# k-flouris/cmf

Measured on AMD Instinct MI355X. Metric: log-density evals/sec (JtJ-cholesky path), MNIST D=784 d=64 bs=512, higher is better.
Workload: dtype f32 (3x3 tangent convs as bf16x3 split MFMA, fp32 accumulate); 1 GPU; C3: MNIST-shaped (1,28,28) uint8-range + U[0,1) noise, non-square flow d=64, cholesky J^T J log-det + g_ij off-diagonal L1 + reconstruction, eval/no_grad; per_gpu_batch=512, global_batch=512, D=784, latent_dimension=64, parallelism=dp1

## Files before the change

cmf_amd/csrc/probe_front.hip:

```cpp
#include <stdint.h>

#include "common.h"

namespace {

constexpr int HID = 64, NT = 256, SLICE = HID * 16;
constexpr int MAXT = 50;
constexpr int MAXCLS = 32;
constexpr int PASS = 64;

__global__ __launch_bounds__(NT) void probe_apply_kernel(cmf_probe_apply_args a, int nitems) {
  __shared__ __attribute__((aligned(16))) float Rs[MAXCLS * HID];
  __shared__ __attribute__((aligned(16))) float Ts[MAXT * PASS];
  __shared__ int tcls[MAXT], toff[MAXT];
  __shared__ int nterm;

  const int per = (nitems + 7) >> 3;
  const int item = (int)(blockIdx.x & 7) * per + (int)(blockIdx.x >> 3);
  if (item >= nitems) return;
  const int H = a.H, W = a.W, HW = H * W;
  const int b = item / HW, p = item - b * HW;
  const int tid = threadIdx.x, lane = tid & 63, wv = tid >> 6;
  const int ncls = a.ns * 16;
  const f32x4 zero = {0.f, 0.f, 0.f, 0.f};

  unsigned long long live = ~0ull;
  if (a.ymask)
    live = *reinterpret_cast<const unsigned long long*>(reinterpret_cast<const unsigned char*>(a.ymask) + (long long)b * a.ymask_np +
                                                        (long long)p * (HID / 8));

  if (wv == 0) {
    int cls = -1, off = 0;
    if (lane < 25 * a.cin) {
      const int w = lane / a.cin, c = lane - w * a.cin;
      const int r = p / W + w / 5 - 2, col = p % W + w % 5 - 2;
      if (r >= 0 && r < H && col >= 0 && col < W) {
        const int q = r * W + col, k = a.cls[c * HW + q];
        if (k >= 0 && k < ncls) {
          cls = k;
          off = (int)(c * a.t_c + q * a.t_px);
        }
      }
    }
    const unsigned long long bal = __ballot(cls >= 0);
    if (cls >= 0) {
      const int pos = __popcll(bal & ((1ull << lane) - 1ull));
      tcls[pos] = cls;
      toff[pos] = off;
    }
    if (lane == 0) nterm = __popcll(bal);
  }

  {
    const int co = tid >> 2, k4 = (tid & 3) * 4;
    const float* rb = a.r + (long long)b * a.r_np + (long long)p * a.r_px + tid * 4;
    for (int s = 0; s < a.ns; ++s) {
      f32x4 v = zero;
      if ((live >> co) & 1) v = *reinterpret_cast<const f32x4*>(rb + s * SLICE);
#pragma unroll
      for (int m = 0; m < 4; ++m) Rs[(s * 16 + k4 + m) * HID + (co & 15) * 4 + (co >> 4)] = v[m];
    }
  }
  __syncthreads();

  const int n = nterm, nsl = a.nc >> 4, cg = lane >> 2, quad = lane & 3;
  const float* tb = a.t + (long long)b * a.t_np;
  for (int s0 = 0; s0 < nsl; s0 += PASS / 16) {
    const int w4 = (nsl - s0 < PASS / 16 ? nsl - s0 : PASS / 16) * 4;
    if (s0) __syncthreads();
    for (int i = tid; i < n * w4; i += NT) {
      const int j = i / w4, x = i - j * w4;
      *reinterpret_cast<f32x4*>(&Ts[j * PASS + 4 * x]) = *reinterpret_cast<const f32x4*>(tb + toff[j] + s0 * 16 + 4 * x);
    }
    __syncthreads();
    const int sl = s0 + wv;
    if (sl >= nsl) continue;
    f32x4 acc[4] = {zero, zero, zero, zero};
    for (int j = 0; j < n; ++j) {
      const f32x4 c4 = *reinterpret_cast<const f32x4*>(&Rs[tcls[j] * HID + cg * 4]);
      const f32x4 t4 = *reinterpret_cast<const f32x4*>(&Ts[j * PASS + wv * 16 + quad * 4]);
#pragma unroll
      for (int i = 0; i < 4; ++i)
#pragma unroll
        for (int k = 0; k < 4; ++k) acc[i][k] = fmaf(c4[i], t4[k], acc[i][k]);
    }
    float* yb = a.y + (long long)b * a.y_np + (long long)p * a.y_px + sl * SLICE + quad * 4;
#pragma unroll
    for (int i = 0; i < 4; ++i) {
      const int co = cg + 16 * i;
      if ((live >> co) & 1) *reinterpret_cast<f32x4*>(yb + co * 16) = acc[i];
    }
  }
}

bool fits_i32(long long v) { return v >= 0 && v <= 0x7fffffffLL; }

}

extern "C" int cmf_probe_apply(const cmf_probe_apply_args* ap, void* stream) {
  if (!ap) return CMF_EINVAL;
  const cmf_probe_apply_args& a = *ap;
  if (!a.r || !a.t || !a.cls || !a.y) return CMF_EINVAL;
  if (a.np <= 0 || a.H <= 0 || a.W <= 0 || a.nc <= 0 || a.nc % 16) return CMF_EINVAL;
  if (a.cin < 1 || 25 * a.cin > MAXT || a.ns < 1 || a.ns * 16 > MAXCLS) return CMF_EINVAL;
  if ((a.r_np | a.r_px | a.t_np | a.t_c | a.t_px | a.y_np | a.y_px) % 4) return CMF_EINVAL;
  if ((uintptr_t)a.r % 16 || (uintptr_t)a.t % 16 || (uintptr_t)a.y % 16) return CMF_EINVAL;
  if (a.r_np < 0 || a.t_np < 0 || a.y_np < 0 || a.t_c < 0) return CMF_EINVAL;
  if (a.r_px < (long long)a.ns * SLICE || a.y_px < (long long)HID * a.nc || a.t_px < a.nc) return CMF_EINVAL;
  const long long HW = (long long)a.H * a.W;
  if (a.ymask && ((uintptr_t)a.ymask % 8 || a.ymask_np % 8 || a.ymask_np < HW * (HID / 8))) return CMF_EINVAL;
  if (HW > (1 << 24) || !fits_i32(a.cin * a.t_c + HW * a.t_px + a.nc)) return CMF_ERANGE;
  const long long nitems = HW * a.np;
  if (nitems > 0x7ffffff0LL) return CMF_ERANGE;
  const int grid = 8 * (int)((nitems + 7) / 8);
  hipLaunchKernelGGL(probe_apply_kernel, dim3(grid), dim3(NT), 0, (hipStream_t)stream, a, (int)nitems);
  CMF_LAUNCH_CHECK();
  return 0;
}
```

Baseline: 1510 evals/s.

## Process horizontal pixel strips per block with shared T band and per-wave pipelining

Restructures the probe-apply kernel so each block handles a strip of 8–16 pixels in a row for one 64-channel pass, instead of one pixel per block. The block loads the 5-row halo band of T and class ids into LDS once and shares it across the strip's pixels. Each wave prefetches the next pixel's R through buffer loads with masked offsets, iterates terms via ballot and readlane, and stores through buffer stores. The kernel is templated on cin/ns and gets occupancy launch bounds. This cuts redundant T/cls loads and per-pixel block overhead, at the cost of more LDS per block and more code complexity.

Result: no change. 1517 evals/s, median of 6 (+0.4%).

```diff
diff --git a/cmf_amd/csrc/probe_front.hip b/cmf_amd/csrc/probe_front.hip
--- a/cmf_amd/csrc/probe_front.hip
+++ b/cmf_amd/csrc/probe_front.hip
@@ -4,92 +4,196 @@
 
 namespace {
 
-constexpr int HID = 64, NT = 256, SLICE = HID * 16;
+constexpr int HID = 64, NT = 256, NW = NT / 64, SLICE = HID * 16;
 constexpr int MAXT = 50;
 constexpr int MAXCLS = 32;
 constexpr int PASS = 64;
-
-__global__ __launch_bounds__(NT) void probe_apply_kernel(cmf_probe_apply_args a, int nitems) {
-  __shared__ __attribute__((aligned(16))) float Rs[MAXCLS * HID];
-  __shared__ __attribute__((aligned(16))) float Ts[MAXT * PASS];
-  __shared__ int tcls[MAXT], toff[MAXT];
-  __shared__ int nterm;
+constexpr int RS_FLAGS = 0x00020000, DROP = 0x7ffffff0;
+constexpr int RROW = HID + 4;
+
+constexpr int strip_of(int cin) { return cin == 1 ? 16 : 8; }
+
+typedef unsigned long long u64;
+typedef unsigned bu32x4 __attribute__((vector_size(16)));
+
+__device__ __forceinline__ auto rsrc_of(const void* p, int bytes) {
+  const u64 u = reinterpret_cast<u64>(p);
+  const unsigned lo = __builtin_amdgcn_readfirstlane((int)(unsigned)u), hi = __builtin_amdgcn_readfirstlane((int)(unsigned)(u >> 32));
+  return __builtin_amdgcn_make_buffer_rsrc(reinterpret_cast<void*>(((u64)hi << 32) | lo), 0, bytes, RS_FLAGS);
+}
+
+__device__ __forceinline__ void wave_lds_fence() {
+  __builtin_amdgcn_fence(__ATOMIC_RELEASE, "wavefront");
+  __builtin_amdgcn_wave_barrier();
+  __builtin_amdgcn_fence(__ATOMIC_ACQUIRE, "wavefront");
+}
+
+__device__ __forceinline__ u64 lane_word(u64 v, int l) {
+  const unsigned lo = __builtin_amdgcn_readlane((int)(unsigned)v, l), hi = __builtin_amdgcn_readlane((int)(unsigned)(v >> 32), l);
+  return ((u64)hi << 32) | lo;
+}
+
+template <int NS>
+__device__ __forceinline__ void fetch_r(f32x4 (&rv)[4 * NS], const float* r, u64 live, bool on, int lane) {
+  const auto rs = rsrc_of(r, on ? NS * SLICE * 4 : 0);
+#pragma unroll
+  for (int s = 0; s < NS; ++s)
+#pragma unroll
+    for (int k = 0; k < 4; ++k)
+      rv[4 * s + k] = __builtin_bit_cast(f32x4, __builtin_amdgcn_raw_buffer_load_b128(
+          rs, (live >> (16 * k + (lane >> 2))) & 1 ? 4 * (s * SLICE + k * 256 + lane * 4) : DROP, 0, 0));
+}
+
+template <int NS>
+__device__ __forceinline__ void write_image(float* Rw, const f32x4 (&rv)[4 * NS], int lane) {
+#pragma unroll
+  for (int s = 0; s < NS; ++s)
+#pragma unroll
+    for (int m = 0; m < 4; ++m) {
+      const f32x4 v = {rv[4 * s][m], rv[4 * s + 1][m], rv[4 * s + 2][m], rv[4 * s + 3][m]};
+      *reinterpret_cast<f32x4*>(&Rw[(s * 16 + (lane & 3) * 4 + m) * RROW + (lane >> 2) * 4]) = v;
+    }
+}
+
+template <int NSL, int CIN, int NS>
+__device__ __forceinline__ void strip_pixels(float* Rw, const float* Tb, const int* bcls, f32x4 (&rv)[4 * NS], u64 words, const float* rb,
+                                             long long r_px, float* yb, long long y_px, int len, int wv, int lane) {
+  constexpr int BAND = strip_of(CIN) + 4;
+  const int cg = lane >> 2, quad = lane & 3;
+  const f32x4 zero = {0.f, 0.f, 0.f, 0.f};
+  write_image<NS>(Rw, rv, lane);
+  for (int x = wv; x < len; x += NW) {
+    const u64 live = lane_word(words, x);
+    const bool more = x + NW < len;
+    wave_lds_fence();
+    fetch_r<NS>(rv, rb + (more ? x + NW : x) * r_px, more ? lane_word(words, x + NW) : 0ull, more, lane);
+
+    int cls = -1, pos = 0;
+    if (lane < 25 * CIN) {
+      const int w = lane / CIN, c = lane - w * CIN;
+      pos = (c * 5 + w / 5) * BAND + x + w % 5;
+      cls = bcls[pos];
+    }
+    const u64 terms = __ballot(cls >= 0);
+
+    f32x4 acc[NSL][4], c4, t4[NSL];
+#pragma unroll
+    for (int s = 0; s < NSL; ++s)
+#pragma unroll
+      for (int i = 0; i < 4; ++i) acc[s][i] = zero;
+    auto read_term = [&](u64& m, f32x4& c, f32x4(&t)[NSL]) {
+      const int l = __builtin_ctzll(m);
+      const int k = __builtin_amdgcn_readlane(cls, l), o = __builtin_amdgcn_readlane(pos, l);
+      m &= m - 1;
+      c = *reinterpret_cast<const f32x4*>(&Rw[k * RROW + cg * 4]);
+#pragma unroll
+      for (int s = 0; s < NSL; ++s) t[s] = *reinterpret_cast<const f32x4*>(&Tb[o * PASS + s * 16 + quad * 4]);
+    };
+    auto add_term = [&]() {
+#pragma unroll
+      for (int s = 0; s < NSL; ++s)
+#pragma unroll
+        for (int i = 0; i < 4; ++i)
+#pragma unroll
+          for (int e = 0; e < 4; ++e) acc[s][i][e] = fmaf(c4[i], t4[s][e], acc[s][i][e]);
+    };
+    if (terms) {
+      u64 m = terms;
+      read_term(m, c4, t4);
+      while (m) {
+        f32x4 cn, tn[NSL];
+        read_term(m, cn, tn);
+        add_term();
+        c4 = cn;
+#pragma unroll
+        for (int s = 0; s < NSL; ++s) t4[s] = tn[s];
+      }
+      add_term();
+    }
+
+    const auto ys = rsrc_of(yb + x * y_px, NSL * SLICE * 4);
+#pragma unroll
+    for (int s = 0; s < NSL; ++s)
+#pragma unroll
+      for (int i = 0; i < 4; ++i) {
+        const int co = cg + 16 * i;
+        __builtin_amdgcn_raw_buffer_store_b128(__builtin_bit_cast(bu32x4, acc[s][i]), ys, (live >> co) & 1 ? 4 * (s * SLICE + co * 16 + quad * 4) : DROP, 0, 0);
+      }
+    wave_lds_fence();
+    write_image<NS>(Rw, rv, lane);
+  }
+}
+
+constexpr int wg_per_cu(int cin, int ns) {
+  return 160 * 1024 / (4 * (cin * 5 * (strip_of(cin) + 4) * (PASS + 1) + NW * 16 * ns * RROW));
+}
+
+template <int CIN, int NS>
+__global__ __launch_bounds__(NT, wg_per_cu(CIN, NS)) void probe_apply_kernel(cmf_probe_apply_args a, int nitems, int spr, int npass) {
+  constexpr int STRIP = strip_of(CIN), BAND = STRIP + 4;
+  constexpr int NPOS = CIN * 5 * BAND, NB = (NPOS + 15) / 16, NCLS = 16 * NS;
+  __shared__ __attribute__((aligned(16))) float Tb[NPOS * PASS];
+  __shared__ __attribute__((aligned(16))) float Rs[NW][NCLS * RROW];
+  __shared__ int bcls[NPOS];
 
   const int per = (nitems + 7) >> 3;
   const int item = (int)(blockIdx.x & 7) * per + (int)(blockIdx.x >> 3);
   if (item >= nitems) return;
   const int H = a.H, W = a.W, HW = H * W;
-  const int b = item / HW, p = item - b * HW;
-  const int tid = threadIdx.x, lane = tid & 63, wv = tid >> 6;
-  const int ncls = a.ns * 16;
-  const f32x4 zero = {0.f, 0.f, 0.f, 0.f};
-
-  unsigned long long live = ~0ull;
-  if (a.ymask)
-    live = *reinterpret_cast<const unsigned long long*>(reinterpret_cast<const unsigned char*>(a.ymask) + (long long)b * a.ymask_np +
-                                                        (long long)p * (HID / 8));
-
-  if (wv == 0) {
-    int cls = -1, off = 0;
-    if (lane < 25 * a.cin) {
-      const int w = lane / a.cin, c = lane - w * a.cin;
-      const int r = p / W + w / 5 - 2, col = p % W + w % 5 - 2;
-      if (r >= 0 && r < H && col >= 0 && col < W) {
-        const int q = r * W + col, k = a.cls[c * HW + q];
-        if (k >= 0 && k < ncls) {
-          cls = k;
-          off = (int)(c * a.t_c + q * a.t_px);
-        }
-      }
-    }
-    const unsigned long long bal = __ballot(cls >= 0);
-    if (cls >= 0) {
-      const int pos = __popcll(bal & ((1ull << lane) - 1ull));
-      tcls[pos] = cls;
-      toff[pos] = off;
-    }
-    if (lane == 0) nterm = __popcll(bal);
-  }
+  const int strip = item / npass, s0 = (item - strip * npass) * (PASS / 16);
+  const int line = strip / spr, x0 = (strip - line * spr) * STRIP;
+  const int b = line / H, row = line - b * H, p0 = row * W + x0;
+  const int len = W - x0 < STRIP ? W - x0 : STRIP;
+  const int tid = threadIdx.x, lane = tid & 63, wv = __builtin_amdgcn_readfirstlane(tid >> 6);
+
+  u64 words = ~0ull;
+  if (a.ymask && lane < len)
+    words = *reinterpret_cast<const u64*>(reinterpret_cast<const unsigned char*>(a.ymask) + (long long)b * a.ymask_np +
+                                          (long long)(p0 + lane) * (HID / 8));
+
+  const float* rb = a.r + (long long)b * a.r_np + (long long)p0 * a.r_px;
+  const int nsl = a.nc >> 4, grp = tid >> 4, l16 = tid & 15;
+  const float* tb = a.t + (long long)b * a.t_np;
+  float* Rw = Rs[wv];
+  const int nslp = nsl - s0 < PASS / 16 ? nsl - s0 : PASS / 16;
+  f32x4 rv[4 * NS];
+  fetch_r<NS>(rv, rb + (wv < len ? wv : 0) * a.r_px, wv < len ? lane_word(words, wv) : 0ull, wv < len, lane);
 
   {
-    const int co = tid >> 2, k4 = (tid & 3) * 4;
-    const float* rb = a.r + (long long)b * a.r_np + (long long)p * a.r_px + tid * 4;
-    for (int s = 0; s < a.ns; ++s) {
-      f32x4 v = zero;
-      if ((live >> co) & 1) v = *reinterpret_cast<const f32x4*>(rb + s * SLICE);
-#pragma unroll
-      for (int m = 0; m < 4; ++m) Rs[(s * 16 + k4 + m) * HID + (co & 15) * 4 + (co >> 4)] = v[m];
+    int off[NB], kk[NB];
+    f32x4 tv[NB];
+#pragma unroll
+    for (int u = 0; u < NB; ++u) {
+      const int pos = grp + 16 * u < NPOS ? grp + 16 * u : NPOS - 1;
+      const int c = pos / (5 * BAND), rem = pos - c * (5 * BAND), r = row + rem / BAND - 2, col = x0 + rem % BAND - 2;
+      kk[u] = a.cls[c * HW + (r >= 0 && r < H && col >= 0 && col < W ? r * W + col : 0)];
+    }
+#pragma unroll
+    for (int u = 0; u < NB; ++u) {
+      const int pos = grp + 16 * u < NPOS ? grp + 16 * u : NPOS - 1;
+      const int c = pos / (5 * BAND), rem = pos - c * (5 * BAND), r = row + rem / BAND - 2, col = x0 + rem % BAND - 2;
+      const bool in = r >= 0 && r < H && col >= 0 && col < W;
+      const int q = in ? r * W + col : 0, k = kk[u];
+      const bool on = in && k >= 0 && k < NCLS;
+      off[u] = on && l16 < 4 * nslp ? (int)(c * a.t_c + q * a.t_px) + s0 * 16 + 4 * l16 : 0;
+      if (l16 == 0) bcls[pos] = on ? k : -1;
+    }
+#pragma unroll
+    for (int u = 0; u < NB; ++u) tv[u] = *reinterpret_cast<const f32x4*>(tb + off[u]);
+#pragma unroll
+    for (int u = 0; u < NB; ++u) {
+      const int pos = grp + 16 * u < NPOS ? grp + 16 * u : NPOS - 1;
+      *reinterpret_cast<f32x4*>(&Tb[pos * PASS + 4 * l16]) = tv[u];
     }
   }
   __syncthreads();
 
-  const int n = nterm, nsl = a.nc >> 4, cg = lane >> 2, quad = lane & 3;
-  const float* tb = a.t + (long long)b * a.t_np;
-  for (int s0 = 0; s0 < nsl; s0 += PASS / 16) {
-    const int w4 = (nsl - s0 < PASS / 16 ? nsl - s0 : PASS / 16) * 4;
-    if (s0) __syncthreads();
-    for (int i = tid; i < n * w4; i += NT) {
-      const int j = i / w4, x = i - j * w4;
-      *reinterpret_cast<f32x4*>(&Ts[j * PASS + 4 * x]) = *reinterpret_cast<const f32x4*>(tb + toff[j] + s0 * 16 + 4 * x);
-    }
-    __syncthreads();
-    const int sl = s0 + wv;
-    if (sl >= nsl) continue;
-    f32x4 acc[4] = {zero, zero, zero, zero};
-    for (int j = 0; j < n; ++j) {
-      const f32x4 c4 = *reinterpret_cast<const f32x4*>(&Rs[tcls[j] * HID + cg * 4]);
-      const f32x4 t4 = *reinterpret_cast<const f32x4*>(&Ts[j * PASS + wv * 16 + quad * 4]);
-#pragma unroll
-      for (int i = 0; i < 4; ++i)
-#pragma unroll
-        for (int k = 0; k < 4; ++k) acc[i][k] = fmaf(c4[i], t4[k], acc[i][k]);
-    }
-    float* yb = a.y + (long long)b * a.y_np + (long long)p * a.y_px + sl * SLICE + quad * 4;
-#pragma unroll
-    for (int i = 0; i < 4; ++i) {
-      const int co = cg + 16 * i;
-      if ((live >> co) & 1) *reinterpret_cast<f32x4*>(yb + co * 16) = acc[i];
-    }
+  float* yb = a.y + (long long)b * a.y_np + (long long)p0 * a.y_px + s0 * SLICE;
+  switch (nslp) {
+    case 4: strip_pixels<4, CIN, NS>(Rw, Tb, bcls, rv, words, rb, a.r_px, yb, a.y_px, len, wv, lane); break;
+    case 3: strip_pixels<3, CIN, NS>(Rw, Tb, bcls, rv, words, rb, a.r_px, yb, a.y_px, len, wv, lane); break;
+    case 2: strip_pixels<2, CIN, NS>(Rw, Tb, bcls, rv, words, rb, a.r_px, yb, a.y_px, len, wv, lane); break;
+    default: strip_pixels<1, CIN, NS>(Rw, Tb, bcls, rv, words, rb, a.r_px, yb, a.y_px, len, wv, lane); break;
   }
 }
 
@@ -110,10 +214,15 @@
   const long long HW = (long long)a.H * a.W;
   if (a.ymask && ((uintptr_t)a.ymask % 8 || a.ymask_np % 8 || a.ymask_np < HW * (HID / 8))) return CMF_EINVAL;
   if (HW > (1 << 24) || !fits_i32(a.cin * a.t_c + HW * a.t_px + a.nc)) return CMF_ERANGE;
-  const long long nitems = HW * a.np;
-  if (nitems > 0x7ffffff0LL) return CMF_ERANGE;
-  const int grid = 8 * (int)((nitems + 7) / 8);
-  hipLaunchKernelGGL(probe_apply_kernel, dim3(grid), dim3(NT), 0, (hipStream_t)stream, a, (int)nitems);
+  if (HW * a.np > 0x7ffffff0LL) return CMF_ERANGE;
+  const int spr = (a.W + strip_of(a.cin) - 1) / strip_of(a.cin);
+  const int npass = (a.nc + PASS - 1) / PASS;
+  const long long n = (long long)a.np * a.H * spr * npass;
+  if (n > 0x7ffffff0LL) return CMF_ERANGE;
+  const int nitems = (int)n, grid = 8 * ((nitems + 7) / 8);
+  auto kernel = a.cin == 1 ? (a.ns == 1 ? probe_apply_kernel<1, 1> : probe_apply_kernel<1, 2>)
+                           : (a.ns == 1 ? probe_apply_kernel<2, 1> : probe_apply_kernel<2, 2>);
+  hipLaunchKernelGGL(kernel, dim3(grid), dim3(NT), 0, (hipStream_t)stream, a, nitems, spr, npass);
   CMF_LAUNCH_CHECK();
   return 0;
 }
```
